# UCSD-Comp-Imaging/Nerf-Simple

Measured on AMD Instinct MI355X. Metric: ray-samples/sec at 800x800x128, higher is better.
Workload: dtype f16

## Files before the change

nerf-simple_amd/csrc/dw_gemm.hip:

```cpp
#include "nerf_device.h"
#include "launchers.h"
#include "dw_products.h"

using namespace nerf_layout;

typedef __bf16 bf16x4 __attribute__((ext_vector_type(4)));

namespace {

constexpr int MAXD = 16;
struct GemmDesc {
    const __bf16* A;
    const __bf16* B;
    float* C;
    int lda, ldb, ldc;
    int M, N;
    int r0, Mv, Nv;
    int wg0, wgs;
    float* bias;
};
struct GemmTable {
    GemmDesc d[MAXD];
    int n;
    long long P;
};

constexpr int SLAB = 32;
static_assert(SLAB == 32, "the slab loop is written for two k-steps");
static_assert(ACT_TILE_PTS % SLAB == 0 && ACT_TILE_PTS * 16 == 4096, "a slab never straddles activation blocks");
constexpr int ROWB = 512;
constexpr int OPB = SLAB * ROWB;
constexpr int KSTEP = 16 * ROWB;
constexpr int SLOTB = 2 * OPB;
constexpr int RING = 4;
constexpr int LDS_BYTES = RING * SLOTB;
constexpr int DMA_PER_SLAB = 2 * SLAB / 2 / 8;

struct Frag { bf16x4 lo, hi; };
template <int KOFF>
__device__ __forceinline__ void read_frag_tr(Frag& f, unsigned addr_lo, unsigned addr_hi) {
    asm volatile("ds_read_b64_tr_b16 %0, %2 offset:%4\n\tds_read_b64_tr_b16 %1, %3 offset:%4"
                 : "=&v"(f.lo), "=&v"(f.hi) : "v"(addr_lo), "v"(addr_hi), "n"(KOFF));
}
__device__ __forceinline__ void frags_landed(Frag (&a)[4], Frag (&b)[2]) {
    asm volatile("s_waitcnt lgkmcnt(0)"
                 : "+v"(a[0].lo), "+v"(a[0].hi), "+v"(a[1].lo), "+v"(a[1].hi), "+v"(a[2].lo), "+v"(a[2].hi),
                   "+v"(a[3].lo), "+v"(a[3].hi), "+v"(b[0].lo), "+v"(b[0].hi), "+v"(b[1].lo), "+v"(b[1].hi));
}
__device__ __forceinline__ bf16x8 whole(const Frag& f) {
    return bf16x8{f.lo[0], f.lo[1], f.lo[2], f.lo[3], f.hi[0], f.hi[1], f.hi[2], f.hi[3]};
}

__global__ __launch_bounds__(512, 2) void dw_gemm_kernel(GemmTable tab) {
    extern __shared__ __attribute__((aligned(16))) char smem[];
    int di;
    dw_product_of_workgroup(tab, di);
    const GemmDesc d = tab.d[di];
    const int slice = blockIdx.x - d.wg0;
    const long long nslab = (tab.P + SLAB - 1) / SLAB;
    const long long s_begin = nslab * slice / d.wgs, s_end = nslab * (slice + 1) / d.wgs;

    const int tid = threadIdx.x, lane = tid & 63;
    const int wave = __builtin_amdgcn_readfirstlane(tid >> 6);
    const int wm = wave >> 2, wn = wave & 3;
    const int m0 = 128 * wm, n0 = 64 * wn;

    const bool pieceA = wave < 4;
    const int pld = pieceA ? d.lda : d.ldb;
    const bool pblk = pld == 0;
    const __bf16* pbase = pieceA ? d.A : d.B;
    const int pwidth = pieceA ? d.M : d.N;
    const long long row_begin = s_begin * SLAB;
    const long long row_end = s_end * SLAB < tab.P ? s_end * SLAB : tab.P;
    const long long slice_rows = row_end > row_begin ? row_end - row_begin : 0;
    const long long slice_blocks = (row_end + ACT_TILE_PTS - 1) / ACT_TILE_PTS - row_begin / ACT_TILE_PTS;
    const __amdgpu_buffer_rsrc_t rs = pblk
        ? __builtin_amdgcn_make_buffer_rsrc(const_cast<char*>(reinterpret_cast<const char*>(pbase))
                                                + (row_begin / ACT_TILE_PTS) * ACT_BLOCK_BYTES,
                                            0, (int)(slice_rows > 0 ? slice_blocks * ACT_BLOCK_BYTES : 0), 0x00020000)
        : __builtin_amdgcn_make_buffer_rsrc(const_cast<__bf16*>(pbase + row_begin * pld), 0,
                                            (int)(slice_rows * pld * 2), 0x00020000);
    constexpr unsigned OUTSIDE = 0xffffffffu;
    unsigned voff[DMA_PER_SLAB];
    unsigned ldst[DMA_PER_SLAB];
    int vrow[DMA_PER_SLAB];
#pragma unroll
    for (int k = 0; k < DMA_PER_SLAB; ++k) {
        const int piece = wave * DMA_PER_SLAB + k, pi = piece & 15;
        ldst[k] = (piece >> 4) * OPB + pi * 1024;
        if (pblk) {
            const int c = 4 * (pi & 7) + (lane >> 4);
            vrow[k] = 16 * (pi >> 3) + ((lane & 15) ^ ((lane >> 4) << 2));
            voff[k] = c * 8 < pwidth ? (unsigned)(c * (ACT_TILE_PTS * 16) + vrow[k] * 16) : OUTSIDE;
        } else {
            vrow[k] = 2 * pi + (lane >> 5);
            const int cg = (lane & 31) ^ ((vrow[k] & 3) << 2);
            voff[k] = cg * 8 < pwidth ? (unsigned)(vrow[k] * pld * 2 + cg * 16) : OUTSIDE;
        }
    }
    auto issue_slab = [&](int it, int slot) {
        const long long p0 = row_begin + (long long)it * SLAB;
        unsigned vadd;
        int rows_left = SLAB;
        if (pblk) {
            vadd = (unsigned)((p0 / ACT_TILE_PTS - row_begin / ACT_TILE_PTS) * ACT_BLOCK_BYTES + (p0 % ACT_TILE_PTS) * 16);
            rows_left = tab.P - p0 < SLAB ? (int)(tab.P - p0) : SLAB;
        } else {
            vadd = (unsigned)it * (unsigned)(SLAB * pld * 2);
        }
#pragma unroll
        for (int k = 0; k < DMA_PER_SLAB; ++k) {
            lds_void* dst = reinterpret_cast<lds_void*>(reinterpret_cast<lds_char*>(0) + slot * SLOTB + ldst[k]);
            const unsigned off = (voff[k] == OUTSIDE || vrow[k] >= rows_left) ? OUTSIDE : voff[k] + vadd;
            __builtin_amdgcn_raw_ptr_buffer_load_lds(rs, dst, 16, off, 0, 0, 2);
        }
    };

    const int grp = lane >> 4, q = (lane & 15) >> 2, pp = lane & 3, h = lane >> 5;
    const int cl = 2 * (grp & 1) + (pp >> 1);
    auto frag_addr = [&](bool blocked, int t, int second) -> unsigned {
        const int r = 8 * h + q + 4 * second;
        if (blocked) return (4 * t + cl) * 256 + ((r ^ (cl << 2)) * 16) + 8 * (pp & 1);
        return r * ROWB + ((((4 * t + cl) ^ ((r & 3) << 2))) * 16) + 8 * (pp & 1);
    };
    unsigned aoff[4][2], boff[2][2];
#pragma unroll
    for (int i = 0; i < 4; ++i)
#pragma unroll
        for (int e = 0; e < 2; ++e) aoff[i][e] = frag_addr(d.lda == 0, m0 / 32 + i, e);
#pragma unroll
    for (int j = 0; j < 2; ++j)
#pragma unroll
        for (int e = 0; e < 2; ++e) boff[j][e] = OPB + frag_addr(d.ldb == 0, n0 / 32 + j, e);

    f32x16 acc[4][2];
#pragma unroll
    for (int i = 0; i < 4; ++i)
#pragma unroll
        for (int j = 0; j < 2; ++j)
#pragma unroll
            for (int r = 0; r < 16; ++r) acc[i][j][r] = 0.f;
    const bool active = m0 < d.M && n0 < d.N;
    float bsum[8] = {0.f, 0.f, 0.f, 0.f, 0.f, 0.f, 0.f, 0.f};
    const int brow = tid & 15, bchunk = tid >> 4;
    const unsigned baddr = bchunk * 256 + ((brow ^ ((bchunk & 3) << 2)) * 16);

#pragma unroll
    for (int k = 0; k < RING - 1; ++k)
        if (s_begin + k < s_end) issue_slab(k, k);
    Frag a0[4], b0[2], a1[4], b1[2];
    auto read_k0 = [&](unsigned base) {
#pragma unroll
        for (int i = 0; i < 4; ++i) read_frag_tr<0>(a0[i], base + aoff[i][0], base + aoff[i][1]);
#pragma unroll
        for (int j = 0; j < 2; ++j) read_frag_tr<0>(b0[j], base + boff[j][0], base + boff[j][1]);
    };
    if (s_begin < s_end) {
        const long long n = s_end - s_begin;
        if (n >= 3) asm volatile("s_waitcnt vmcnt(8)" ::: "memory");
        else if (n == 2) asm volatile("s_waitcnt vmcnt(4)" ::: "memory");
        else asm volatile("s_waitcnt vmcnt(0)" ::: "memory");
        __builtin_amdgcn_s_barrier();
        if (active) read_k0(0);
    }
    for (long long s = s_begin; s < s_end; ++s) {
        const int it = (int)(s - s_begin), slot = it & (RING - 1);
        const long long left = s_end - s;
        const unsigned base = slot * SLOTB;
        if (active) {
            frags_landed(a0, b0);
#pragma unroll
            for (int i = 0; i < 4; ++i) read_frag_tr<KSTEP>(a1[i], base + aoff[i][0], base + aoff[i][1]);
#pragma unroll
            for (int j = 0; j < 2; ++j) read_frag_tr<KSTEP>(b1[j], base + boff[j][0], base + boff[j][1]);
            __builtin_amdgcn_sched_barrier(0);
#pragma unroll
            for (int i = 0; i < 4; ++i)
#pragma unroll
                for (int j = 0; j < 2; ++j)
                    acc[i][j] = __builtin_amdgcn_mfma_f32_32x32x16_bf16(whole(a0[i]), whole(b0[j]), acc[i][j], 0, 0, 0);
            __builtin_amdgcn_sched_barrier(0);
        }
        if (left >= 2) {
            if (left >= 3) asm volatile("s_waitcnt vmcnt(4)" ::: "memory");
            else asm volatile("s_waitcnt vmcnt(0)" ::: "memory");
            __builtin_amdgcn_s_barrier();
            if (s + RING - 1 < s_end) issue_slab(it + RING - 1, (it + RING - 1) & (RING - 1));
        }
        if (active) {
            frags_landed(a1, b1);
            if (left >= 2) read_k0(((it + 1) & (RING - 1)) * SLOTB);
            __builtin_amdgcn_sched_barrier(0);
#pragma unroll
            for (int i = 0; i < 4; ++i)
#pragma unroll
                for (int j = 0; j < 2; ++j)
                    acc[i][j] = __builtin_amdgcn_mfma_f32_32x32x16_bf16(whole(a1[i]), whole(b1[j]), acc[i][j], 0, 0, 0);
        }
        if (d.bias && bchunk * 8 < d.M) {
#pragma unroll
            for (int ks = 0; ks < SLAB / 16; ++ks) {
                const bf16x8 v = *reinterpret_cast<const __attribute__((address_space(3))) bf16x8*>(
                    reinterpret_cast<lds_char*>(0) + base + ks * KSTEP + baddr);
#pragma unroll
                for (int k = 0; k < 8; ++k) bsum[k] += (float)v[k];
            }
        }
    }
    __syncthreads();
    if (d.bias && bchunk * 8 < d.M && s_begin < s_end) {
        float* red = reinterpret_cast<float*>(smem);
#pragma unroll
        for (int k = 0; k < 8; ++k) red[(brow * 32 + bchunk) * 8 + k] = bsum[k];
    }
    __syncthreads();
    if (d.bias && s_begin < s_end && tid < d.M) {
        const int ch = tid >> 3, k = tid & 7;
        float v = 0.f;
        for (int r = 0; r < 16; ++r) v += reinterpret_cast<float*>(smem)[(r * 32 + ch) * 8 + k];
        atomicAdd(d.bias + tid, v);
    }
    if (active && s_begin < s_end) {
#pragma unroll
        for (int i = 0; i < 4; ++i)
#pragma unroll
            for (int j = 0; j < 2; ++j)
#pragma unroll
                for (int r = 0; r < 16; ++r) {
                    const int row = m0 + 32 * i + (r & 3) + 8 * (r >> 2) + 4 * h - d.r0;
                    const int col = n0 + 32 * j + (lane & 31);
                    if (row >= 0 && row < d.Mv && col < d.Nv)
                        atomicAdd(d.C + (long long)row * d.ldc + col, acc[i][j][r]);
                }
    }
}

__global__ __launch_bounds__(256) void pack_draw_kernel(const float* __restrict__ d_raw, __bf16* __restrict__ dsr,
                                                        long long P, float* __restrict__ g_rgb_b,
                                                        float* __restrict__ g_sig_b) {
    __shared__ float red[4][4];
    f32x4 s = {0.f, 0.f, 0.f, 0.f};
    const __bf16 z = (__bf16)0.f;
    for (long long p = blockIdx.x * (long long)blockDim.x + threadIdx.x; p < P; p += (long long)gridDim.x * blockDim.x) {
        const f32x4 d = *reinterpret_cast<const f32x4*>(d_raw + p * 4);
        s += d;
        bf16x8* o = reinterpret_cast<bf16x8*>(dsr + p * 32);
        o[0] = bf16x8{(__bf16)d[0], (__bf16)d[1], (__bf16)d[2], (__bf16)d[3], z, z, z, z};
        o[1] = bf16x8{z, z, z, z, z, z, z, z};
        o[2] = o[1];
        o[3] = o[1];
    }
#pragma unroll
    for (int k = 0; k < 4; ++k) {
        float v = s[k];
#pragma unroll
        for (int off = 32; off >= 1; off >>= 1) v += __shfl_xor(v, off);
        if ((threadIdx.x & 63) == 0) red[threadIdx.x >> 6][k] = v;
    }
    __syncthreads();
    if (threadIdx.x < 4) {
        const float v = red[0][threadIdx.x] + red[1][threadIdx.x] + red[2][threadIdx.x] + red[3][threadIdx.x];
        atomicAdd(threadIdx.x < 3 ? g_rgb_b + threadIdx.x : g_sig_b, v);
    }
}

__global__ __launch_bounds__(256) void zero_f32_kernel(float* __restrict__ p, long long n) {
    const long long i = (blockIdx.x * (long long)blockDim.x + threadIdx.x) * 4;
    if (i + 3 < n) *reinterpret_cast<f32x4*>(p + i) = f32x4{0.f, 0.f, 0.f, 0.f};
    else for (long long k = i; k < n; ++k) p[k] = 0.f;
}

}

extern "C" int nerf_amd_launch_param_gradients_begin(const float* d_raw, void* scratch, float* grads, long long P,
                                                     hipStream_t stream) {
    (void)hipGetLastError();
    static_assert(PARAM_COUNT % 4 == 0, "16-byte zero fill");
    hipLaunchKernelGGL(zero_f32_kernel, dim3((PARAM_COUNT / 4 + 255) / 256), dim3(256), 0, stream, grads,
                       (long long)PARAM_COUNT);
    hipError_t e = hipGetLastError();
    if (e != hipSuccess) return (int)e;
    if (P <= 0) return 0;
    hipLaunchKernelGGL(pack_draw_kernel, dim3(512), dim3(256), 0, stream, d_raw, reinterpret_cast<__bf16*>(scratch), P,
                       grads + OFF_C1_B, grads + OFF_SIG_B);
    return (int)hipGetLastError();
}

extern "C" int nerf_amd_launch_param_gradients_finish(const void* acts_v, const void* dys_v, const void* posx64_v,
                                                      const void* posd32_v, const void* scratch, float* grads,
                                                      long long P, int bucket, hipStream_t stream) {
    (void)hipGetLastError();
    hipError_t e = hipSuccess;
    if (P <= 0) return 0;
    const __bf16* acts = reinterpret_cast<const __bf16*>(acts_v);
    const __bf16* dys = reinterpret_cast<const __bf16*>(dys_v);
    const __bf16* posx = reinterpret_cast<const __bf16*>(posx64_v);
    const __bf16* posd = reinterpret_cast<const __bf16*>(posd32_v);
    const __bf16* dsr = reinterpret_cast<const __bf16*>(scratch);
    struct Operand { const __bf16* p; int ld, width; };
    auto operand = [&](DwOperand o) -> Operand {
        const int w = dw_operand_width(o, DW_BF16);
        if (o.kind == DwKind::DY || o.kind == DwKind::ACT)
            return {(o.kind == DwKind::DY ? dys : acts) + act_offset_bytes(o.layer, P) / 2, 0, w};
        return {o.kind == DwKind::POSX ? posx : o.kind == DwKind::POSD ? posd : dsr, w, w};
    };
    const DwPlan plan = dw_plan(DW_BF16, P, bucket, device_cus());
    GemmTable t{};
    t.P = P;
    t.n = plan.n;
    for (int i = 0; i < plan.n; ++i) {
        const DwProduct& p = DW_PRODUCTS[plan.product[i]];
        const Operand A = operand(p.a), B = operand(p.b);
        GemmDesc& g = t.d[i];
        g.A = A.p; g.lda = A.ld; g.M = A.width; g.B = B.p; g.ldb = B.ld; g.N = B.width;
        g.C = grads + p.coff; g.ldc = p.ldc; g.r0 = p.r0; g.Mv = p.Mv; g.Nv = p.Nv;
        g.bias = p.boff >= 0 ? grads + p.boff : nullptr;
        g.wg0 = plan.wg0[i]; g.wgs = plan.wgs[i];
    }
    e = allow_dynamic_lds(reinterpret_cast<const void*>(dw_gemm_kernel), LDS_BYTES);
    if (e != hipSuccess) return (int)e;
    hipLaunchKernelGGL(dw_gemm_kernel, dim3(plan.workgroups), dim3(512), LDS_BYTES, stream, t);
    return (int)hipGetLastError();
}

extern "C" int nerf_amd_launch_param_gradients(const float* d_raw, const void* acts_v, const void* dys_v,
                                               const void* posx64_v, const void* posd32_v, void* scratch,
                                               float* grads, long long P, hipStream_t stream) {
    const int rc = nerf_amd_launch_param_gradients_begin(d_raw, scratch, grads, P, stream);
    if (rc) return rc;
    return nerf_amd_launch_param_gradients_finish(acts_v, dys_v, posx64_v, posd32_v, scratch, grads, P, 0, stream);
}
```

nerf-simple_amd/csrc/dw_products.h:

```cpp
#pragma once
#include "nerf_layout.h"

namespace nerf_layout {

enum class DwKind { DY, ACT, POSX, POSD, DSR };
struct DwOperand { DwKind kind; int layer; };
struct DwProduct { DwOperand a, b; int coff, ldc, r0, Mv, Nv, boff; };
constexpr int DW_NUM_PRODUCTS = 14;
constexpr DwOperand dw_dy(int L) { return {DwKind::DY, L}; }
constexpr DwOperand dw_act(int L) { return {DwKind::ACT, L}; }
constexpr DwOperand DW_POSX{DwKind::POSX, 0}, DW_POSD{DwKind::POSD, 0}, DW_DSR{DwKind::DSR, 0};
constexpr DwProduct dw_dense(int L, int w_off) { return {dw_dy(L), dw_act(L - 1), w_off, 256, 0, 256, 256, w_off + 65536}; }
constexpr int DW_LW = 256 * 256 + 256;
constexpr DwProduct DW_PRODUCTS[DW_NUM_PRODUCTS] = {
    {dw_dy(0), DW_POSX, OFF_L0_W, 63, 0, 256, 63, OFF_L0_B},
    dw_dense(1, OFF_L1_W), dw_dense(2, OFF_L1_W + DW_LW),
    dw_dense(3, OFF_L1_W + 2 * DW_LW), dw_dense(4, OFF_L1_W + 3 * DW_LW),
    {dw_dy(5), dw_act(4), OFF_SKIP_W, 319, 0, 256, 256, OFF_SKIP_B},
    {dw_dy(5), DW_POSX, OFF_SKIP_W + 256, 319, 0, 256, 63, -1},
    dw_dense(6, OFF_L6_W), dw_dense(7, OFF_L6_W + DW_LW),
    {DW_DSR, dw_act(7), OFF_SIG_W, 256, 3, 1, 256, -1},
    {dw_dy(8), dw_act(7), OFF_L2_W, 256, 0, 256, 256, OFF_L2_B},
    {dw_dy(9), dw_act(8), OFF_C0_W, 283, 0, 128, 256, OFF_C0_B},
    {dw_dy(9), DW_POSD, OFF_C0_W + 256, 283, 0, 128, 27, -1},
    {DW_DSR, dw_act(9), OFF_C1_W, 128, 0, 3, 128, -1},
};

struct DwForm { int slab, bytes_per_feature, dsr_width; };
constexpr DwForm DW_BF16{32, 2, 32}, DW_E4M3{64, 1, 16};
constexpr int dw_operand_width(DwOperand o, DwForm f) {
    return o.kind == DwKind::POSX ? 64 : o.kind == DwKind::POSD ? 32 : o.kind == DwKind::DSR ? f.dsr_width : act_width(o.layer);
}

struct DwPlan { int n; int product[16]; int wg0[16]; int wgs[16]; int workgroups; };
static inline DwPlan dw_plan(DwForm f, long long P, int bucket, int cus) {
    DwPlan plan{};
    int width[16];
    for (int i = 0; i < DW_NUM_PRODUCTS; ++i) {
        const bool head = DW_PRODUCTS[i].coff < GRAD_BUCKET_SPLIT;
        if (bucket != 0 && head != (bucket == 2)) continue;
        width[plan.n] = dw_operand_width(DW_PRODUCTS[i].a, f) + dw_operand_width(DW_PRODUCTS[i].b, f);
        plan.product[plan.n++] = i;
    }
    const int n = plan.n;
    constexpr double slab_cost = 1024.0;
    double total = 0;
    for (int i = 0; i < n; ++i) total += (double)width[i] + slab_cost;
    const long long nslab = (P + f.slab - 1) / f.slab;
    const long long need = (P * 256 * f.bytes_per_feature >> 30) + 1;
    long long w[16];
    double rem[16];
    long long used = 0;
    for (int i = 0; i < n; ++i) {
        const double share = ((double)width[i] + slab_cost) / total * cus;
        w[i] = (long long)share;
        rem[i] = share - (double)w[i];
        if (w[i] < need) { w[i] = need; rem[i] = 0; }
        if (w[i] >= nslab) { w[i] = nslab; rem[i] = -1; }
        used += w[i];
    }
    while (used < cus) {
        int best = -1;
        for (int i = 0; i < n; ++i)
            if (rem[i] >= 0 && w[i] < nslab && (best < 0 || rem[i] > rem[best])) best = i;
        if (best < 0) break;
        ++w[best]; rem[best] = 0; ++used;
    }
    for (int i = 0; i < n; ++i) {
        plan.wg0[i] = plan.workgroups;
        plan.wgs[i] = (int)w[i];
        plan.workgroups += (int)w[i];
    }
    return plan;
}

struct F8Scratch { long long px, pd, ds, total; };
constexpr F8Scratch f8_scratch(long long P) {
    const long long pd = align256(f8_narrow_bytes(dw_operand_width(DW_POSX, DW_E4M3), P));
    const long long ds = pd + align256(f8_narrow_bytes(dw_operand_width(DW_POSD, DW_E4M3), P));
    return {0, pd, ds, ds + align256(f8_narrow_bytes(dw_operand_width(DW_DSR, DW_E4M3), P))};
}

#if defined(__HIPCC__)
template <class Table>
__device__ __forceinline__ void dw_product_of_workgroup(const Table& tab, int& di) {
    di = 0;
    while (di + 1 < tab.n && (int)blockIdx.x >= tab.d[di + 1].wg0) ++di;
}
#endif

}
```

Baseline: 1.350 billion.

## Fold small weight-gradient products into carrier GEMMs sharing an operand

After: 1.345 billion. Within noise of the previous version (-0.4%).

```diff
diff --git a/nerf-simple_amd/csrc/dw_gemm.hip b/nerf-simple_amd/csrc/dw_gemm.hip
--- a/nerf-simple_amd/csrc/dw_gemm.hip
+++ b/nerf-simple_amd/csrc/dw_gemm.hip
@@ -18,7 +18,13 @@
     int r0, Mv, Nv;
     int wg0, wgs;
     float* bias;
+    const __bf16* R;
+    float* RC;
+    int rkind;
+    int rcol, rldc, rNv;
 };
+enum { RIDER_NONE = 0, RIDER_COLSUM = 1, RIDER_TILES = 2 };
+constexpr int RIDER_W = 32;
 struct GemmTable {
     GemmDesc d[MAXD];
     int n;
@@ -33,8 +39,13 @@
 constexpr int KSTEP = 16 * ROWB;
 constexpr int SLOTB = 2 * OPB;
 constexpr int RING = 4;
-constexpr int LDS_BYTES = RING * SLOTB;
+constexpr int RIDB = SLAB * RIDER_W * 2;
+constexpr int RID0 = RING * SLOTB;
+constexpr int LDS_BYTES = RING * (SLOTB + RIDB);
 constexpr int DMA_PER_SLAB = 2 * SLAB / 2 / 8;
+constexpr int DMA_WAIT = DMA_PER_SLAB + 1;
+static_assert(RIDB == 8 * 64 * 4, "one 4-byte piece per wave covers a rider slab");
+static_assert(LDS_BYTES <= 160 * 1024, "one workgroup per CU");
 
 struct Frag { bf16x4 lo, hi; };
 template <int KOFF>
@@ -46,6 +57,14 @@
     asm volatile("s_waitcnt lgkmcnt(0)"
                  : "+v"(a[0].lo), "+v"(a[0].hi), "+v"(a[1].lo), "+v"(a[1].hi), "+v"(a[2].lo), "+v"(a[2].hi),
                    "+v"(a[3].lo), "+v"(a[3].hi), "+v"(b[0].lo), "+v"(b[0].hi), "+v"(b[1].lo), "+v"(b[1].hi));
+}
+__device__ __forceinline__ void frags_landed(Frag& a, Frag& b, Frag& c, Frag& e) {
+    asm volatile("s_waitcnt lgkmcnt(0)"
+                 : "+v"(a.lo), "+v"(a.hi), "+v"(b.lo), "+v"(b.hi), "+v"(c.lo), "+v"(c.hi), "+v"(e.lo), "+v"(e.hi));
+}
+template <int N>
+__device__ __forceinline__ void dma_wait() {
+    asm volatile("s_waitcnt vmcnt(%0)" ::"n"(N) : "memory");
 }
 __device__ __forceinline__ bf16x8 whole(const Frag& f) {
     return bf16x8{f.lo[0], f.lo[1], f.lo[2], f.lo[3], f.hi[0], f.hi[1], f.hi[2], f.hi[3]};
@@ -98,6 +117,11 @@
             voff[k] = cg * 8 < pwidth ? (unsigned)(vrow[k] * pld * 2 + cg * 16) : OUTSIDE;
         }
     }
+    const __amdgpu_buffer_rsrc_t rr = __builtin_amdgcn_make_buffer_rsrc(
+        const_cast<__bf16*>(d.R + (d.rkind != RIDER_NONE ? row_begin * RIDER_W : 0)), 0,
+        (int)(d.rkind != RIDER_NONE ? slice_rows * (RIDER_W * 2) : 0), 0x00020000);
+    const unsigned roff = d.rkind == RIDER_TILES ? (unsigned)(wave * 256 + lane * 4)
+                        : d.rkind == RIDER_COLSUM && tid < SLAB ? (unsigned)(tid * (RIDER_W * 2) + ((d.rcol * 2) & ~3)) : OUTSIDE;
     auto issue_slab = [&](int it, int slot) {
         const long long p0 = row_begin + (long long)it * SLAB;
         unsigned vadd;
@@ -114,6 +138,8 @@
             const unsigned off = (voff[k] == OUTSIDE || vrow[k] >= rows_left) ? OUTSIDE : voff[k] + vadd;
             __builtin_amdgcn_raw_ptr_buffer_load_lds(rs, dst, 16, off, 0, 0, 2);
         }
+        lds_void* rdst = reinterpret_cast<lds_void*>(reinterpret_cast<lds_char*>(0) + RID0 + slot * RIDB + wave * 256);
+        __builtin_amdgcn_raw_ptr_buffer_load_lds(rr, rdst, 4, roff == OUTSIDE ? OUTSIDE : roff + (unsigned)it * (unsigned)RIDB, 0, 0, 2);
     };
 
     const int grp = lane >> 4, q = (lane & 15) >> 2, pp = lane & 3, h = lane >> 5;
@@ -141,6 +167,14 @@
 #pragma unroll
             for (int r = 0; r < 16; ++r) acc[i][j][r] = 0.f;
     const bool active = m0 < d.M && n0 < d.N;
+    const bool tiles = d.rkind == RIDER_TILES && wm == 1 && !active && 32 * wn < d.M;
+    unsigned raoff[2], rboff[2];
+#pragma unroll
+    for (int e = 0; e < 2; ++e) {
+        raoff[e] = frag_addr(d.lda == 0, wn, e);
+        rboff[e] = RID0 + (8 * h + q + 4 * e) * (RIDER_W * 2) + cl * 16 + 8 * (pp & 1);
+    }
+    float rsum[8] = {0.f, 0.f, 0.f, 0.f, 0.f, 0.f, 0.f, 0.f};
     float bsum[8] = {0.f, 0.f, 0.f, 0.f, 0.f, 0.f, 0.f, 0.f};
     const int brow = tid & 15, bchunk = tid >> 4;
     const unsigned baddr = bchunk * 256 + ((brow ^ ((bchunk & 3) << 2)) * 16);
@@ -157,9 +191,9 @@
     };
     if (s_begin < s_end) {
         const long long n = s_end - s_begin;
-        if (n >= 3) asm volatile("s_waitcnt vmcnt(8)" ::: "memory");
-        else if (n == 2) asm volatile("s_waitcnt vmcnt(4)" ::: "memory");
-        else asm volatile("s_waitcnt vmcnt(0)" ::: "memory");
+        if (n >= 3) dma_wait<2 * DMA_WAIT>();
+        else if (n == 2) dma_wait<DMA_WAIT>();
+        else dma_wait<0>();
         __builtin_amdgcn_s_barrier();
         if (active) read_k0(0);
     }
@@ -182,8 +216,8 @@
             __builtin_amdgcn_sched_barrier(0);
         }
         if (left >= 2) {
-            if (left >= 3) asm volatile("s_waitcnt vmcnt(4)" ::: "memory");
-            else asm volatile("s_waitcnt vmcnt(0)" ::: "memory");
+            if (left >= 3) dma_wait<DMA_WAIT>();
+            else dma_wait<0>();
             __builtin_amdgcn_s_barrier();
             if (s + RING - 1 < s_end) issue_slab(it + RING - 1, (it + RING - 1) & (RING - 1));
         }
@@ -196,6 +230,27 @@
 #pragma unroll
                 for (int j = 0; j < 2; ++j)
                     acc[i][j] = __builtin_amdgcn_mfma_f32_32x32x16_bf16(whole(a1[i]), whole(b1[j]), acc[i][j], 0, 0, 0);
+        }
+        if (tiles) {
+            const unsigned rbase = slot * RIDB;
+            read_frag_tr<0>(a0[0], base + raoff[0], base + raoff[1]);
+            read_frag_tr<0>(b0[0], rbase + rboff[0], rbase + rboff[1]);
+            read_frag_tr<KSTEP>(a1[0], base + raoff[0], base + raoff[1]);
+            read_frag_tr<16 * RIDER_W * 2>(b1[0], rbase + rboff[0], rbase + rboff[1]);
+            frags_landed(a0[0], b0[0], a1[0], b1[0]);
+            acc[0][0] = __builtin_amdgcn_mfma_f32_32x32x16_bf16(whole(a0[0]), whole(b0[0]), acc[0][0], 0, 0, 0);
+            acc[0][0] = __builtin_amdgcn_mfma_f32_32x32x16_bf16(whole(a1[0]), whole(b1[0]), acc[0][0], 0, 0, 0);
+        }
+        if (d.rkind == RIDER_COLSUM && bchunk * 8 < d.N) {
+#pragma unroll
+            for (int ks = 0; ks < SLAB / 16; ++ks) {
+                const bf16x8 v = *reinterpret_cast<const __attribute__((address_space(3))) bf16x8*>(
+                    reinterpret_cast<lds_char*>(0) + base + OPB + ks * KSTEP + baddr);
+                const float w = (float)*reinterpret_cast<const __attribute__((address_space(3))) __bf16*>(
+                    reinterpret_cast<lds_char*>(0) + RID0 + slot * RIDB + (16 * ks + brow) * 4 + (d.rcol & 1) * 2);
+#pragma unroll
+                for (int k = 0; k < 8; ++k) rsum[k] = __builtin_fmaf(w, (float)v[k], rsum[k]);
+            }
         }
         if (d.bias && bchunk * 8 < d.M) {
 #pragma unroll
@@ -219,6 +274,29 @@
         float v = 0.f;
         for (int r = 0; r < 16; ++r) v += reinterpret_cast<float*>(smem)[(r * 32 + ch) * 8 + k];
         atomicAdd(d.bias + tid, v);
+    }
+    if (d.rkind == RIDER_COLSUM && s_begin < s_end) {
+        float* red = reinterpret_cast<float*>(smem);
+        __syncthreads();
+        if (bchunk * 8 < d.N) {
+#pragma unroll
+            for (int k = 0; k < 8; ++k) red[(brow * 32 + bchunk) * 8 + k] = rsum[k];
+        }
+        __syncthreads();
+        if (tid < d.N && tid < d.rNv) {
+            const int ch = tid >> 3, k = tid & 7;
+            float v = 0.f;
+            for (int r = 0; r < 16; ++r) v += red[(r * 32 + ch) * 8 + k];
+            atomicAdd(d.RC + tid, v);
+        }
+    }
+    if (tiles && s_begin < s_end) {
+#pragma unroll
+        for (int r = 0; r < 16; ++r) {
+            const int row = 32 * wn + (r & 3) + 8 * (r >> 2) + 4 * h;
+            const int col = lane & 31;
+            if (row < d.M && col < d.rNv) atomicAdd(d.RC + (long long)row * d.rldc + col, acc[0][0][r]);
+        }
     }
     if (active && s_begin < s_end) {
 #pragma unroll
@@ -304,7 +382,7 @@
             return {(o.kind == DwKind::DY ? dys : acts) + act_offset_bytes(o.layer, P) / 2, 0, w};
         return {o.kind == DwKind::POSX ? posx : o.kind == DwKind::POSD ? posd : dsr, w, w};
     };
-    const DwPlan plan = dw_plan(DW_BF16, P, bucket, device_cus());
+    const DwPlan plan = dw_plan_riders(DW_BF16, P, bucket, device_cus());
     GemmTable t{};
     t.P = P;
     t.n = plan.n;
@@ -316,6 +394,17 @@
         g.C = grads + p.coff; g.ldc = p.ldc; g.r0 = p.r0; g.Mv = p.Mv; g.Nv = p.Nv;
         g.bias = p.boff >= 0 ? grads + p.boff : nullptr;
         g.wg0 = plan.wg0[i]; g.wgs = plan.wgs[i];
+        const int r = dw_rider_carried_by(plan.product[i]);
+        if (r >= 0) {
+            const DwProduct& q = DW_PRODUCTS[DW_RIDERS[r].product];
+            const Operand R = operand(DW_RIDERS[r].operand);
+            const bool colsum = dw_same(q.b, p.b);
+            if (R.ld != RIDER_W || (colsum ? q.Mv != 1 || B.ld != 0 || q.Nv > B.width
+                                           : q.r0 != 0 || q.Mv != A.width || A.width > 128 || q.Nv > RIDER_W || !dw_same(q.a, p.a)))
+                return (int)hipErrorInvalidValue;
+            g.R = R.p; g.RC = grads + q.coff; g.rkind = colsum ? RIDER_COLSUM : RIDER_TILES;
+            g.rcol = q.r0; g.rldc = q.ldc; g.rNv = q.Nv;
+        }
     }
     e = allow_dynamic_lds(reinterpret_cast<const void*>(dw_gemm_kernel), LDS_BYTES);
     if (e != hipSuccess) return (int)e;
diff --git a/nerf-simple_amd/csrc/dw_products.h b/nerf-simple_amd/csrc/dw_products.h
--- a/nerf-simple_amd/csrc/dw_products.h
+++ b/nerf-simple_amd/csrc/dw_products.h
@@ -74,6 +74,68 @@
     return plan;
 }
 
+struct DwRider { int product, carrier; DwOperand operand; };
+constexpr int DW_NUM_RIDERS = 2;
+constexpr DwRider DW_RIDERS[DW_NUM_RIDERS] = {{9, 10, DW_DSR}, {12, 11, DW_POSD}};
+constexpr bool dw_same(DwOperand x, DwOperand y) { return x.kind == y.kind && x.layer == y.layer; }
+static_assert(dw_same(DW_PRODUCTS[9].a, DW_DSR) && dw_same(DW_PRODUCTS[9].b, DW_PRODUCTS[10].b), "the sigma head shares layers_2's B");
+static_assert(dw_same(DW_PRODUCTS[12].b, DW_POSD) && dw_same(DW_PRODUCTS[12].a, DW_PRODUCTS[11].a), "the d part shares the h part's A");
+static_assert(DW_PRODUCTS[9].coff >= GRAD_BUCKET_SPLIT && DW_PRODUCTS[10].coff >= GRAD_BUCKET_SPLIT &&
+              DW_PRODUCTS[11].coff >= GRAD_BUCKET_SPLIT && DW_PRODUCTS[12].coff >= GRAD_BUCKET_SPLIT, "riders and carriers share a bucket");
+constexpr int dw_rider_carried_by(int i) {
+    for (int r = 0; r < DW_NUM_RIDERS; ++r) if (DW_RIDERS[r].carrier == i) return r;
+    return -1;
+}
+constexpr int dw_rider_index(int i) {
+    for (int r = 0; r < DW_NUM_RIDERS; ++r) if (DW_RIDERS[r].product == i) return r;
+    return -1;
+}
+constexpr int dw_rider_plan_width(int i, DwForm f) {
+    if (dw_rider_index(i) >= 0) return 0;
+    const int r = dw_rider_carried_by(i);
+    return dw_operand_width(DW_PRODUCTS[i].a, f) + dw_operand_width(DW_PRODUCTS[i].b, f) + (r >= 0 ? dw_operand_width(DW_RIDERS[r].operand, f) : 0);
+}
+static inline DwPlan dw_plan_riders(DwForm f, long long P, int bucket, int cus) {
+    DwPlan plan{};
+    int width[16];
+    for (int i = 0; i < DW_NUM_PRODUCTS; ++i) {
+        const bool head = DW_PRODUCTS[i].coff < GRAD_BUCKET_SPLIT;
+        if ((bucket != 0 && head != (bucket == 2)) || dw_rider_index(i) >= 0) continue;
+        width[plan.n] = dw_rider_plan_width(i, f);
+        plan.product[plan.n++] = i;
+    }
+    const int n = plan.n;
+    constexpr double slab_cost = 1024.0;
+    double total = 0;
+    for (int i = 0; i < n; ++i) total += (double)width[i] + slab_cost;
+    const long long nslab = (P + f.slab - 1) / f.slab;
+    const long long need = (P * 256 * f.bytes_per_feature >> 30) + 1;
+    long long w[16];
+    double rem[16];
+    long long used = 0;
+    for (int i = 0; i < n; ++i) {
+        const double share = ((double)width[i] + slab_cost) / total * cus;
+        w[i] = (long long)share;
+        rem[i] = share - (double)w[i];
+        if (w[i] < need) { w[i] = need; rem[i] = 0; }
+        if (w[i] >= nslab) { w[i] = nslab; rem[i] = -1; }
+        used += w[i];
+    }
+    while (used < cus) {
+        int best = -1;
+        for (int i = 0; i < n; ++i)
+            if (rem[i] >= 0 && w[i] < nslab && (best < 0 || rem[i] > rem[best])) best = i;
+        if (best < 0) break;
+        ++w[best]; rem[best] = 0; ++used;
+    }
+    for (int i = 0; i < n; ++i) {
+        plan.wg0[i] = plan.workgroups;
+        plan.wgs[i] = (int)w[i];
+        plan.workgroups += (int)w[i];
+    }
+    return plan;
+}
+
 struct F8Scratch { long long px, pd, ds, total; };
 constexpr F8Scratch f8_scratch(long long P) {
     const long long pd = align256(f8_narrow_bytes(dw_operand_width(DW_POSX, DW_E4M3), P));
```
